# xiangli0608/Creating-2D-laser-slam-from-scratch

Measured on AMD Instinct MI355X. Metric: scan-matches/sec (1081-beam vs 2000x2000 grid), higher is better.
Workload: dtype u8

## Files before the change

### creating-2d-laser-slam-from-scratch_amd/api.py

```python
from __future__ import annotations

import ctypes as C
import os
import sys
import math
import weakref

import numpy as np

from . import build as _build

LSLAM_OK = 0
ERRORS = {
    -1: "LSLAM_ERR_INVALID_ARGUMENT",
    -2: "LSLAM_ERR_NO_DEVICE",
    -3: "LSLAM_ERR_INDEX_OUT_OF_RANGE",
    -4: "LSLAM_ERR_PROBABILITY_SEARCH",
    -5: "LSLAM_ERR_NO_BEST_POSE",
    -6: "LSLAM_ERR_HIP",
    -7: "LSLAM_ERR_SMEAR_DEVIATION",
    -8: "LSLAM_ERR_UNSUPPORTED",
}


# ... 218 lines not shown
    return LaserParams(laser.angle_min, laser.angle_max, laser.angle_increment, laser.range_min,
                       laser.range_max, range_threshold, *offset)


_LIB = None


def lib() -> C.CDLL:
    global _LIB
    if _LIB is not None:
        return _LIB
    path = os.environ.get("LSLAM_GPU_LIB") or _build.build_library()
    L = C.CDLL(str(path))
    vp, i32, dbl = C.c_void_p, C.c_int, C.c_double
    L.lslam_abi_version.restype = i32
    L.lslam_create.argtypes = [i32, C.POINTER(vp)]
    L.lslam_destroy.argtypes = [vp]
    L.lslam_last_error.restype = C.c_char_p
    L.lslam_last_error.argtypes = [vp]
    L.lslam_synchronize.argtypes = [vp]
    L.lslam_stream.restype = vp
    L.lslam_stream.argtypes = [vp]
    L.lslam_dev_alloc.argtypes = [vp, C.c_size_t, C.POINTER(vp)]
    L.lslam_dev_free.argtypes = [vp, vp]
    L.lslam_dev_upload.argtypes = [vp, vp, vp, C.c_size_t]
    L.lslam_dev_download.argtypes = [vp, vp, vp, C.c_size_t]
    L.lslam_profile_enable.argtypes = [vp, i32]
    L.lslam_profile_only.argtypes = [vp, C.c_char_p]
    L.lslam_profile_reset.argtypes = [vp]
    L.lslam_profile_read.argtypes = [vp, vp, i32]
    L.lslam_matcher_config_defaults.argtypes = [C.POINTER(MatcherConfig)]
    L.lslam_matcher_config_defaults.restype = None
    L.lslam_matcher_create.argtypes = [vp, C.POINTER(MatcherConfig), C.POINTER(LaserParams), C.POINTER(vp)]
    L.lslam_matcher_destroy.argtypes = [vp]
    L.lslam_matcher_destroy.restype = None
    L.lslam_matcher_num_beams.argtypes = [vp]
    L.lslam_matcher_grid_info.argtypes = [vp, vp, vp]
    L.lslam_matcher_get_grid_u8.argtypes = [vp, vp]
    L.lslam_matcher_get_kernel_u8.argtypes = [vp, vp]
    L.lslam_matcher_set_grid_u8.argtypes = [vp, vp, vp]
    L.lslam_matcher_set_grid_u8_dev.argtypes = [vp, vp, vp]
    L.lslam_matcher_grid_dev_ptr.restype = vp
    L.lslam_matcher_grid_dev_ptr.argtypes = [vp]
    L.lslam_sensor_pose_from_robot.argtypes = [C.POINTER(LaserParams), vp, vp]
    L.lslam_sensor_pose_from_robot.restype = None
    L.lslam_robot_pose_from_sensor.argtypes = [C.POINTER(LaserParams), vp, vp]
    L.lslam_robot_pose_from_sensor.restype = None
    L.lslam_matcher_set_base_scans.argtypes = [vp, i32, vp, i32, vp, vp]
    L.lslam_matcher_match_scan.argtypes = [vp, i32, vp, i32, vp, vp, vp, i32, i32, vp]
    L.lslam_matcher_match_batch.argtypes = [vp, i32, vp, i32, vp, i32, i32, vp]
    L.lslam_matcher_match_batch_dev_f32.argtypes = [vp, i32, vp, i32, vp, i32, i32, vp]
    L.lslam_matcher_match_batch_dev_f64.argtypes = [vp, i32, vp, i32, vp, i32, i32, vp]
    L.lslam_matcher_debug_lookup_table.argtypes = [vp, vp, vp, dbl, dbl, dbl, vp, C.POINTER(i32)]
    L.lslam_matcher_debug_coarse_sums.argtypes = [vp, vp, vp, vp, C.POINTER(i32), C.POINTER(i32),
                                                  C.POINTER(i32), i32]
    L.lslam_matcher_debug_coarse_sums_batch.argtypes = [vp, i32, vp, i32, vp, vp]
    L.lslam_matcher_debug_fine_sums_batch.argtypes = [vp, i32, vp, i32, vp, vp, vp, C.POINTER(i32), C.POINTER(i32), C.POINTER(i32)]
    L.lslam_matcher_debug_valid_mask.argtypes = [vp, vp, vp, vp, vp]
    L.lslam_frontend_create.argtypes = [vp, i32, dbl, dbl, dbl, C.POINTER(vp)]
    L.lslam_frontend_destroy.argtypes = [vp]
    L.lslam_frontend_destroy.restype = None
    L.lslam_frontend_reset.argtypes = [vp]
    L.lslam_frontend_process.argtypes = [vp, vp, i32, vp, C.POINTER(i32), vp, vp, C.POINTER(dbl)]
    L.lslam_frontend_running_scans.argtypes = [vp]
    L.lslam_frontend_config_defaults.argtypes = [C.POINTER(FrontEndConfig)]
    L.lslam_frontend_config_defaults.restype = None
# ... 1285 lines not shown
```

### creating-2d-laser-slam-from-scratch_amd/csrc/scan_matcher.hip

```cpp
#include <algorithm>
#include <atomic>
#include <chrono>
#include <cmath>
#include <cstdlib>
#include <cstring>
#include <type_traits>
#include <vector>

#include "common.hpp"
#include "karto_math.hpp"

using namespace lslam;

#if defined(LSLAM_EXP_SERIAL_PRIO)
#define LSLAM_SERIAL_BEGIN() __builtin_amdgcn_s_setprio(3)
#define LSLAM_SERIAL_END() __builtin_amdgcn_s_setprio(0)
#else
#define LSLAM_SERIAL_BEGIN()
#define LSLAM_SERIAL_END()
#endif

namespace {

LSLAM_STAMP_TABLE(g_sm_stamps)
// ... 965 lines not shown
  }
#pragma unroll
  for (int q = 0; q < kTile3Angles; q++) {
    uint32_t tot[9];
    tot[0] = wave_sum(e0[q] & 0xFFFFu), tot[1] = wave_sum(o01[q] & 0xFFFFu), tot[2] = wave_sum(e0[q] >> 16);
    tot[3] = wave_sum(e1[q] & 0xFFFFu), tot[4] = wave_sum(o01[q] >> 16), tot[5] = wave_sum(e1[q] >> 16);
    tot[6] = wave_sum(e2[q] & 0xFFFFu), tot[7] = wave_sum(o2[q]), tot[8] = wave_sum(e2[q] >> 16);
    uint32_t mine = 0;
#pragma unroll
    for (int c = 0; c < 9; c++)
      if (lane == c) mine = tot[c];
    if (lane < 9 && angle_on[q]) r_scan[(a0 + q) * 9 + lane] = (int32_t)mine;
  }
}

template <int kTile3Angles>
__global__ void __launch_bounds__(64)
k_resp_tile3(const uint4* __restrict__ tiles, int tile_cols, Geom g, PassCfg pc, const Lattice* __restrict__ lat,
             const double2* __restrict__ cossin, const double2* __restrict__ local, int32_t* __restrict__ resp, size_t resp_stride, int S) {
  const int w = blockIdx.x;
  const int xcd = w & 7, r = w >> 3;
  const int pairs = (pc.na + kTile3Angles - 1) / kTile3Angles;
  const int s = (r / pairs) * 8 + xcd;
  const int a0 = (r % pairs) * kTile3Angles;
  if (s >= S) return;
  resp_tile3_wave<kTile3Angles>(s, a0, (int)threadIdx.x, tiles, tile_cols, g, pc, lat, cossin, local, resp + (size_t)s * resp_stride);
}

constexpr int kPosChunk = 16;
#if !defined(LSLAM_TUNE_REDUCE_NARROW_MIN)
#define LSLAM_TUNE_REDUCE_NARROW_MIN 2048
#endif
constexpr int kReduceNarrowMinScans = LSLAM_TUNE_REDUCE_NARROW_MIN;
__device__ __forceinline__ void generic_item(const uint8_t* __restrict__ grid, const Geom& g, const PassCfg& pc,
                                             const Lattice& L, const double2* __restrict__ lp, int32_t* r, int a,
                                             int c, int lane) {
  const int np = pc.nx * pc.ny;
  const double angle = (L.center[2] - pc.ang_off) + (uint32_t)a * pc.ang_res;
  const double cosine = cos(angle), sine = sin(angle);
  int pos[kPosChunk];
#pragma unroll
  for (int q = 0; q < kPosChunk; q++) {
    int f = c * kPosChunk + q;
    pos[q] = f < np ? L.gx[f % pc.nx] + L.gy[f / pc.nx] * g.stride : -1;
  }
  int32_t acc[kPosChunk];
#pragma unroll
  for (int q = 0; q < kPosChunk; q++) acc[q] = 0;
  for (int b = lane; b < g.n_beams; b += 64) {
    double2 p = lp[b];
    if (isnan(p.x)) continue;
    int t = lookup_offset(p.x, p.y, cosine, sine, g.off_x, g.off_y, g.scale, g.stride);
#pragma unroll
    for (int q = 0; q < kPosChunk; q++) {
      long long idx = (long long)pos[q] + t;
      if (pos[q] >= 0 && idx >= 0 && idx < g.data_size) acc[q] += grid[idx];
    }
  }
#pragma unroll
  for (int q = 0; q < kPosChunk; q++) {
    int v = acc[q];
    for (int o = 32; o > 0; o >>= 1) v += __shfl_xor(v, o);
    int f = c * kPosChunk + q;
    if (lane == 0 && f < np) r[(size_t)a * np + f] = v;
  }
}

__global__ void __launch_bounds__(64)
k_resp_generic(const uint8_t* __restrict__ grid, Geom g, PassCfg pc, const Lattice* __restrict__ lat,
               const double2* __restrict__ local, int32_t* __restrict__ resp, size_t resp_stride, int S) {
  const int chunks = (pc.nx * pc.ny + kPosChunk - 1) / kPosChunk;
  const int per_scan = pc.na * chunks;
  const long long total = (long long)S * per_scan;
  for (long long w = blockIdx.x; w < total; w += gridDim.x) {
    const int s = (int)(w / per_scan), rem = (int)(w % per_scan);
    const Lattice& L = lat[s];
    if (!L.active || L.status != 0) continue;
    generic_item(grid, g, pc, L, local + (size_t)s * g.n_beams, resp + (size_t)s * resp_stride, rem / chunks,
                 rem % chunks, threadIdx.x);
  }
}

__device__ __forceinline__ void block_generic_fallback(const uint8_t* __restrict__ grid, const Geom& g,
                                                       const PassCfg& pc, const Lattice& L,
                                                       const double2* __restrict__ lp, int32_t* r, int fb_step,
                                                       int tid, int nthreads) {
  if (fb_step == 0 || (L.step_x == fb_step && L.step_y == fb_step)) return;
  const int chunks = (pc.nx * pc.ny + kPosChunk - 1) / kPosChunk;
  const int per_scan = pc.na * chunks;
  for (int w = tid >> 6; w < per_scan; w += nthreads >> 6) generic_item(grid, g, pc, L, lp, r, w / chunks, w % chunks, tid & 63);
  __syncthreads();
}

struct Cand {
  double x, y, angle;
};

__device__ __forceinline__ Cand cand_of(int k, const PassCfg& pc, const double* center) {
  int a = k % pc.na, c = k / pc.na;
  int xi = c % pc.nx, yi = c / pc.nx;
  Cand cd;
  cd.x = -pc.off_x + (uint32_t)xi * pc.res_x;
  cd.y = -pc.off_y + (uint32_t)yi * pc.res_y;
  cd.angle = (center[2] - pc.ang_off) + (uint32_t)a * pc.ang_res;
  return cd;
}

__device__ __forceinline__ double penalized(int32_t sum, const Cand& cd, const double* center, int n_beams,
                                            const SearchCfg& sc) {
  double r = response_of_sum(sum, n_beams, sc);
  if (sc.do_penalize && !double_equal(r, 0.0)) {
    double sd = ksq(cd.x) + ksq(cd.y);
    double dp = 1.0 - (kDistPenaltyGain * sd / sc.dvp);
    dp = dp > sc.min_dp ? dp : sc.min_dp;
    double sad = ksq(cd.angle - center[2]);
    double ap = 1.0 - (kAnglePenaltyGain * sad / sc.avp);
    ap = ap > sc.min_ap ? ap : sc.min_ap;
    r *= (dp * ap);
  }
  return r;
}

__device__ __forceinline__ double block_max(double v, double* sh, int tid, int nthreads) {
// ... 142 lines not shown
      cov[0] = kMaxVariance; cov[4] = kMaxVariance; cov[8] = 4 * ksq(pc.ang_res);
    } else {
      double axx = 0, axy = 0, ayy = 0, norm = 0;
      for (int c = 0; c < ncand; c++) {
        double rr = terms[4 * c];
        if (rr >= (best - 0.1)) {
          norm += rr;
          axx += terms[4 * c + 1];
          axy += terms[4 * c + 2];
          ayy += terms[4 * c + 3];
        }
      }
      if (norm > kTol) {
        double vxx = axx / norm, vxy = axy / norm, vyy = ayy / norm;
        double vthth = 4 * ksq(pc.ang_res);
        double min_xx = 0.1 * ksq(pc.res_x), min_yy = 0.1 * ksq(pc.res_y);
        vxx = vxx > min_xx ? vxx : min_xx;
        vyy = vyy > min_yy ? vyy : min_yy;
        double mult = 1.0 / best;
        cov[0] = vxx * mult; cov[1] = vxy * mult; cov[3] = vxy * mult; cov[4] = vyy * mult;
        cov[8] = vthth;
      }
      if (double_equal(cov[0], 0.0)) cov[0] = kMaxVariance;
      if (double_equal(cov[4], 0.0)) cov[4] = kMaxVariance;
    }
  }
  o.mean[0] = avg[0]; o.mean[1] = avg[1]; o.mean[2] = avg[2];
  for (int i = 0; i < 9; i++) o.cov[i] = cov[i];
  o.best = best > 1.0 ? 1.0 : best;
  o.expand = (use_expansion && o.status == 0 && pass_index < 3 && double_equal(o.best, 0.0)) ? 1 : 0;
  out[s] = o;
}

template <int NT>
__device__ __forceinline__ void reduce_coarse_lds_block(
    const int s, const int tid, const Geom& g, const PassCfg& pc, const SearchCfg& sc, Lattice* lat, int32_t* r,
    CoarseOut* __restrict__ out, int use_expansion, int pass_index, const uint8_t* __restrict__ grid,
    const double2* __restrict__ local, int fb_step, const PassCfg& fine_pc, double2* fine_cossin, int fine_step,
    int zero_fine_words, int parts, unsigned char* smem) {
  __shared__ double sh[NT];
  __shared__ double s_ap[kMaxAngles];
  __shared__ unsigned long long s_nz[4];
  __shared__ double s_avg[3];
  __shared__ int s_status, s_bad, s_ntie, s_wcnt[(NT + 63) / 64];
  const Lattice& L = lat[s];
  if (!L.active) return;
  if (L.status != 0) {
    if (tid == 0) { out[s].status = L.status; out[s].expand = 0; out[s].best = 0.0; }
    return;
  }
  LSLAM_PHASE_CLOCK(pck);
  block_generic_fallback(grid, g, pc, L, local + (size_t)s * g.n_beams, r, fb_step, tid, NT);
  const int ncand = pc.nx * pc.ny;
  const int total = ncand * pc.na;
  const int words = (total + 31) / 32;
  double* latmax = (double*)smem;
  double* probs = latmax + (size_t)parts * ncand;
  double* terms = probs + g.probs_side * g.probs_side;
  uint32_t* mask = (uint32_t*)(terms + 4 * ncand);
  int* cell = (int*)(mask + words);
  int* tie = cell + ncand;
  double* dpen = terms;
  const double center[3] = {L.center[0], L.center[1], L.center[2]};

  const double p_off_x = center[0] - pc.off_x, p_off_y = center[1] - pc.off_y;
  if (tid == 0) { s_bad = 0; s_ntie = 0; }
  for (int c = tid; c < ncand; c += NT) {
    const int xi = c % pc.nx, yi = c / pc.nx;
    const double x = -pc.off_x + (uint32_t)xi * pc.res_x;
    const double y = -pc.off_y + (uint32_t)yi * pc.res_y;
    const double sd = ksq(x) + ksq(y);
    double dp = 1.0 - (kDistPenaltyGain * sd / sc.dvp);
    dpen[c] = dp > sc.min_dp ? dp : sc.min_dp;
    const double wx = center[0] + x, wy = center[1] + y;
    const int gx = world_to_grid(wx, p_off_x, g.scale), gy = world_to_grid(wy, p_off_y, g.scale);
    cell[c] = (gx < 0 || gx >= g.probs_side || gy < 0 || gy >= g.probs_side) ? -1 : gy * g.probs_side + gx;
  }
  for (int a = tid; a < pc.na; a += NT) {
    const double angle = (center[2] - pc.ang_off) + (uint32_t)a * pc.ang_res;
    const double sad = ksq(angle - center[2]);
    double ap = 1.0 - (kAnglePenaltyGain * sad / sc.avp);
    s_ap[a] = ap > sc.min_ap ? ap : sc.min_ap;
  }
  for (int wd = tid; wd < words; wd += NT) mask[wd] = 0u;
  for (int c = tid; c < g.probs_side * g.probs_side; c += NT) probs[c] = 0.0;
  __syncthreads();
  LSLAM_PHASE_MARK(pck, 0);

  auto value_of = [&](int32_t sum, int c, int a) -> double {
    double v = response_of_sum(sum, g.n_beams, sc);
    if (sc.do_penalize && !double_equal(v, 0.0)) v *= (dpen[c] * s_ap[a]);
    return v;
  };
  double lm = -1.0;
  for (int idx = tid; idx < ncand * parts; idx += NT) {
    const int part = idx / ncand, c = idx - part * ncand;
    const int a_lo = part * pc.na / parts, a_hi = (part + 1) * pc.na / parts;
    double m = -1.0;
#if !defined(LSLAM_TUNE_REDUCE_BATCH)
#define LSLAM_TUNE_REDUCE_BATCH 11
#endif
    constexpr int kBatch = LSLAM_TUNE_REDUCE_BATCH;
    for (int a0 = a_lo; a0 < a_hi; a0 += kBatch) {
      int32_t rv[kBatch];
#pragma unroll
      for (int i = 0; i < kBatch; i++) rv[i] = a0 + i < a_hi ? r[(a0 + i) * ncand + c] : 0;
#pragma unroll
      for (int i = 0; i < kBatch; i++)
        if (a0 + i < a_hi) {
          const double v = value_of(rv[i], c, a0 + i);
          m = m > v ? m : v;
        }
    }
    latmax[(size_t)part * ncand + c] = m;
    lm = lm > m ? lm : m;
  }
  LSLAM_PHASE_MARK(pck, 1);
  const double best = block_max(lm, sh, tid, NT);
  LSLAM_PHASE_MARK(pck, 2);

  for (int c = tid; c < ncand; c += NT) {
    double m = latmax[c];
    for (int q = 1; q < parts; q++) m = m > latmax[(size_t)q * ncand + c] ? m : latmax[(size_t)q * ncand + c];
    latmax[c] = m;
    if (cell[c] < 0) s_bad = 1;
    else atomicMax((unsigned long long*)&probs[cell[c]], (unsigned long long)__double_as_longlong(m < 0.0 ? 0.0 : m));
    if (!(m + 2.0 * kTol < best)) tie[atomicAdd(&s_ntie, 1)] = c;
  }
  __syncthreads();
  for (int idx = tid, n = s_ntie * pc.na; idx < n; idx += NT) {
    const int c = tie[idx / pc.na], a = idx % pc.na;
    if (double_equal(value_of(r[a * ncand + c], c, a), best)) {
      const int k = c * pc.na + a;
      atomicOr(&mask[k >> 5], 1u << (k & 31));
    }
  }
  __syncthreads();
  for (int w0 = 0; w0 < 256; w0 += NT) {
    const int wd = w0 + tid;
    const unsigned long long nz = __ballot(wd < words && mask[wd] != 0u);
    if ((tid & 63) == 0 && wd < 256) s_nz[wd >> 6] = nz;
  }
  __syncthreads();
  LSLAM_PHASE_MARK(pck, 3);
  if (tid == 0) {
    LSLAM_SERIAL_BEGIN();
    int st = s_bad ? LSLAM_ERR_PROBABILITY_SEARCH : 0;
    double avg[3] = {0, 0, 0};
    if (st == 0) {
      double ax = 0, ay = 0, tx = 0, ty = 0;
      int cnt = 0;
      for (int wv = 0; wv < 4; wv++) {
        unsigned long long nzw = s_nz[wv];
        while (nzw) {
          const int wd = wv * 64 + (__ffsll((long long)nzw) - 1);
          nzw &= nzw - 1;
          uint32_t m = mask[wd];
          while (m) {
            const int bit = __ffs(m) - 1;
            m &= m - 1;
            const Cand cd = cand_of(wd * 32 + bit, pc, center);
            const double h = normalize_angle(cd.angle);
            ax += center[0] + cd.x;
            ay += center[1] + cd.y;
            double sn, cs;
            sincos(h, &sn, &cs);
            tx += cs;
            ty += sn;
            cnt++;
          }
        }
      }
      if (cnt == 0) {
        st = LSLAM_ERR_NO_BEST_POSE;
      } else {
        ax /= cnt; ay /= cnt; tx /= cnt; ty /= cnt;
        avg[0] = ax; avg[1] = ay; avg[2] = atan2(ty, tx);
      }
    }
    s_avg[0] = avg[0]; s_avg[1] = avg[1]; s_avg[2] = avg[2];
    s_status = st;
    LSLAM_SERIAL_END();
  }
  __syncthreads();
  LSLAM_PHASE_MARK(pck, 4);
  if (fine_cossin != nullptr && tid >= NT - 64) {
    const double center2[3] = {s_avg[0], s_avg[1], s_avg[2]};
    pass_setup_wave(s, tid - (NT - 64), g, fine_pc, center2, s_status == 0, lat, fine_cossin, fine_step);
  }
  const double dx = s_avg[0] - center[0], dy = s_avg[1] - center[1];
  const double thr = best - 0.1;
  int n_pass = 0;
  for (int c0 = 0; c0 < ncand; c0 += NT) {
    const int c = c0 + tid;
    double rr = 0.0, t1 = 0.0, t2 = 0.0, t3 = 0.0;
    bool pass = false;
    if (c < ncand) {
      const int xi = c % pc.nx, yi = c / pc.nx;
      const double x = -pc.off_x + (uint32_t)xi * pc.res_x;
      const double y = -pc.off_y + (uint32_t)yi * pc.res_y;
      rr = cell[c] >= 0 ? probs[cell[c]] : 0.0;
      t1 = (ksq(x - dx) * rr);
      t2 = ((x - dx) * (y - dy) * rr);
      t3 = (ksq(y - dy) * rr);
      pass = rr >= thr;
    }
    const unsigned long long bal = __ballot(pass);
    if ((tid & 63) == 0) s_wcnt[tid >> 6] = __popcll(bal);
    __syncthreads();
    int off = n_pass;
    for (int w = 0; w < (tid >> 6); w++) off += s_wcnt[w];
    for (int w = 0; w < (NT + 63) / 64; w++) n_pass += s_wcnt[w];
    if (pass) {
      const int k = off + __popcll(bal & ((1ull << (tid & 63)) - 1ull));
      terms[4 * k + 0] = rr; terms[4 * k + 1] = t1; terms[4 * k + 2] = t2; terms[4 * k + 3] = t3;
    }
    __syncthreads();
  }
  LSLAM_PHASE_MARK(pck, 5);
  if (tid == 0) {
    CoarseOut o;
    o.status = s_status;
    o.flags = pass_index > 0 ? 1 : 0;
    o.pad = 0;
    const double avg[3] = {s_avg[0], s_avg[1], s_avg[2]};
    double cov[9] = {1, 0, 0, 0, 1, 0, 0, 0, 1};
    if (o.status == 0) {
      if (best < kTol) {
        cov[0] = kMaxVariance; cov[4] = kMaxVariance; cov[8] = 4 * ksq(pc.ang_res);
      } else {
        double axx = 0, axy = 0, ayy = 0, norm = 0;
        int c = 0;
        for (; c + 4 <= n_pass; c += 4) {
          double q[16];
  #pragma unroll
          for (int i = 0; i < 16; i++) q[i] = terms[4 * c + i];
  #pragma unroll
          for (int i = 0; i < 4; i++) { norm += q[4 * i]; axx += q[4 * i + 1]; axy += q[4 * i + 2]; ayy += q[4 * i + 3]; }
        }
        for (; c < n_pass; c++) { norm += terms[4 * c]; axx += terms[4 * c + 1]; axy += terms[4 * c + 2]; ayy += terms[4 * c + 3]; }
        if (norm > kTol) {
          double vxx = axx / norm, vxy = axy / norm, vyy = ayy / norm;
          double vthth = 4 * ksq(pc.ang_res);
          double min_xx = 0.1 * ksq(pc.res_x), min_yy = 0.1 * ksq(pc.res_y);
          vxx = vxx > min_xx ? vxx : min_xx;
          vyy = vyy > min_yy ? vyy : min_yy;
          double mult = 1.0 / best;
          cov[0] = vxx * mult; cov[1] = vxy * mult; cov[3] = vxy * mult; cov[4] = vyy * mult;
          cov[8] = vthth;
        }
        if (double_equal(cov[0], 0.0)) cov[0] = kMaxVariance;
        if (double_equal(cov[4], 0.0)) cov[4] = kMaxVariance;
      }
    }
    o.mean[0] = avg[0]; o.mean[1] = avg[1]; o.mean[2] = avg[2];
    for (int i = 0; i < 9; i++) o.cov[i] = cov[i];
    o.best = best > 1.0 ? 1.0 : best;
    o.expand = (use_expansion && o.status == 0 && pass_index < 3 && double_equal(o.best, 0.0)) ? 1 : 0;
    out[s] = o;
  }
  for (int i = tid; i < zero_fine_words; i += NT) r[i] = 0;
  LSLAM_PHASE_MARK(pck, 6);
  LSLAM_PHASE_FLUSH(pck, g_sm_stamps, 3, (unsigned)(s * (NT >> 6) + (tid >> 6)), (tid & 63) == 0);
}

struct SpecArgs {
  const double* ranges;
  double pose[3];
  int* out;
  const double2* local;
};
__device__ __forceinline__ void anchor_spec_block(int n, const SpecArgs& sa, const Geom& g, unsigned char* smem);
template <int NT>
__global__ void __launch_bounds__(NT)
k_reduce_coarse_lds(Geom g, PassCfg pc, SearchCfg sc, Lattice* lat,
                    int32_t* resp, size_t resp_stride, CoarseOut* __restrict__ out,
                    int use_expansion, int pass_index, const uint8_t* __restrict__ grid,
                const double2* __restrict__ local, int fb_step, PassCfg fine_pc,
                    double2* fine_cossin, int fine_step, int zero_fine_words, int parts, SpecArgs spec) {
  extern __shared__ __align__(16) unsigned char smem[];
  if constexpr (NT == 1024) {
    if (spec.out && blockIdx.x + 1 == gridDim.x) {
      anchor_spec_block(g.n_beams, spec, g, smem);
      return;
    }
  }
  reduce_coarse_lds_block<NT>((int)blockIdx.x, (int)threadIdx.x, g, pc, sc, lat, resp + (size_t)blockIdx.x * resp_stride, out,
                              use_expansion, pass_index, grid, local, fb_step, fine_pc, fine_cossin, fine_step, zero_fine_words,
                              parts, smem);
}


__global__ void __launch_bounds__(256)
k_table_big(int S, Geom g, PassCfg pc, const Lattice* __restrict__ lat, const double2* __restrict__ local,
            int32_t* __restrict__ tbl, unsigned long long* __restrict__ best_bits) {
  const int b = blockIdx.x * blockDim.x + threadIdx.x;
  const int a = blockIdx.y, s = blockIdx.z;
  if (b == 0 && a == 0) best_bits[s] = 0ull;
  if (b >= g.n_beams) return;
  const Lattice& L = lat[s];
  int32_t v = kInvalidScan;
  if (L.active && L.status == 0) {
    const double angle = (L.center[2] - pc.ang_off) + (uint32_t)a * pc.ang_res;
    const double2 p = local[(size_t)s * g.n_beams + b];
    if (!isnan(p.x)) v = lookup_offset(p.x, p.y, cos(angle), sin(angle), g.off_x, g.off_y, g.scale, g.stride);
  }
  tbl[((size_t)s * pc.na + a) * g.n_beams + b] = v;
// ... 1566 lines not shown
  ~BusyGuard() {
    if (ok) m->busy.store(false);
  }
};
#define LSLAM_NOT_REENTRANT(m)                                                                                   \
  BusyGuard busy_guard(m);                                                                                       \
  if (!busy_guard.ok)                                                                                            \
    return (m)->ctx->fail(LSLAM_ERR_INVALID_ARGUMENT, "matcher used concurrently: a ScanMatcher instance is not " \
                                                      "re-entrant (one grid + one set of workspaces, Mapper.h:1273-1278)")

void arm_done_ticket(lslam_matcher* m) {
  if (!m->h_done) {
    if (hipHostMalloc((void**)&m->h_done, sizeof(int), hipHostMallocDefault) != hipSuccess) {
      (void)hipGetLastError();
      m->h_done = nullptr;
      return;
    }
    *m->h_done = 0;
  }
  m->arm_next = true;
}
int wait_record(lslam_matcher* m) {
  lslam_context* ctx = m->ctx;
  if (m->done_armed) {
    m->done_armed = false;
    if (spin_for_ticket(m->h_done, m->done_ticket)) return LSLAM_OK;
  }
  LSLAM_HIP(ctx, hipStreamSynchronize(ctx->stream));
  return LSLAM_OK;
}

int n_angles_of(double off, double res) { return lattice_count(off, res); }

PassCfg coarse_pass_cfg(const lslam_matcher* m, const Geom& g) {
  const double res = 1.0 / g.scale;
  PassCfg pc;
  pc.off_x = pc.off_y = 0.5 * ((double)g.probs_side - 1) * res;
  pc.res_x = pc.res_y = 2 * res;
  pc.ang_off = m->cfg.coarse_search_angle_offset;
  pc.ang_res = m->cfg.coarse_angle_resolution;
  pc.nx = lattice_count(pc.off_x, pc.res_x);
  pc.ny = lattice_count(pc.off_y, pc.res_y);
  pc.na = n_angles_of(pc.ang_off, pc.ang_res);
  pc.mode = 0;
  return pc;
}

template <typename RT>
int match_batch_impl(lslam_matcher* m, int S, const RT* d_ranges, int stride, const double* d_poses,
                     int do_penalize, int do_refine, lslam_match_result* d_out,
                     int32_t* dbg_coarse_sums , int force_generic) {
  lslam_context* ctx = m->ctx;
  if (!m->pipe_in_step) {
    int jrc = pipe_join(m);
    if (jrc) return jrc;
  }
  Geom g = m->g;
  const bool prep_was_done = m->prep_done;
  size_t prezeroed = m->resp_prezeroed;
  m->prep_done = false;
  m->resp_prezeroed = 0;
  int* done_flag = nullptr;
  int done_ticket = 0;
  m->done_armed = false;
  if (m->arm_next && S == 1 && S < kReduceNarrowMinScans && m->h_done) {
    done_flag = m->h_done;
    done_ticket = ++m->done_ticket;
    m->done_armed = true;
  }
  m->arm_next = false;
  const SpecArgs spec_req = m->spec_armed ? m->spec_req : SpecArgs{};
  m->spec_armed = false;
  m->spec_launched = false;
  if (S <= 0) return LSLAM_OK;
  LSLAM_HIP(ctx, hipSetDevice(ctx->device));
  if (g.n_beams == 0) {
    m->done_armed = false;
    launch(ctx, "result_no_readings", k_result_no_readings, dim3((S + 255) / 256), dim3(256), 0, S,
           d_poses, m->cfg.coarse_angle_resolution, d_out);
// ... 82 lines not shown
      m->ptile_dirty = false;
    }
    return true;
  };
  auto tiles4_possible = [&]() -> bool {
    return g.n_beams <= 16384 && !m->tile_failed &&
           (unsigned long long)g.data_size * 4ull + (1ull << 24) < (1ull << 32);
  };
  auto ensure_tiles4 = [&]() -> bool {
    if (!tiles4_possible()) return false;
    if (!m->d_tiles) {
      m->tile_cols = g.stride / 2;
      m->tile_rows = (g.height + 1) / 2 + kTileYPad / 2 + 1;
      m->tile_rows += m->tile_rows & 1;
      if (hipMalloc((void**)&m->d_tiles, (size_t)((m->tile_cols + 3) / 4) * 4 * m->tile_rows * sizeof(uint4)) != hipSuccess) {
        (void)hipGetLastError();
        m->d_tiles = nullptr;
        m->tile_failed = true;
        return false;
      }
    }
    if (m->tile_dirty) {
      launch(ctx, "tile4", k_tile4, dim3((m->tile_cols + 255) / 256, m->tile_rows), dim3(256), 0,
             (const uint8_t*)m->d_grid, g.stride, g.data_size, m->d_tiles, m->tile_cols, m->tile_rows);
      m->tile_dirty = false;
    }
    return true;
  };
  auto reduce_lds = [&](const PassCfg& p, bool cache) -> size_t {
    size_t total = (size_t)p.nx * p.ny * p.na;
    return (cache ? total * 8 : 0) + (size_t)p.nx * p.ny * (8 + 32 + 4) + (size_t)g.probs_side * g.probs_side * 8 +
           ((total + 31) / 32) * 4 + 16;
  };
  auto reduce_parts = [&](const PassCfg& p, int nt) -> int { return std::max(1, std::min(8, nt / (p.nx * p.ny))); };
  auto reduce_lds_nocache = [&](const PassCfg& p, int parts) -> size_t {
    size_t total = (size_t)p.nx * p.ny * p.na;
    return (size_t)p.nx * p.ny * (8 * parts + 32 + 4 + 4) + (size_t)g.probs_side * g.probs_side * 8 + ((total + 31) / 32) * 4 + 16;
  };
  int fb_step = 0;
  bool fine_prezeroed = false;
  auto run_responses = [&](const PassCfg& p, int step, const char* name) -> int {
    const int variant = force_generic ? 0 : (p.nx <= 4 && p.ny <= 4) ? 1 : (p.nx <= 12) ? 2 : (p.nx <= 16) ? 3 : 0;
    fb_step = variant ? step : 0;
    if (!setup_done)
      launch(ctx, "pass_setup", k_pass_setup, dim3(S), dim3(64), 0, S, g, p, d_poses,
             (const CoarseOut*)m->d_coarse.p, m->d_lat.p, m->d_cossin.p, step);
    setup_done = false;
    const long long waves = (long long)((S + 7) / 8) * 8 * p.na;
    bool tiled = variant == 1 && step == 1 && p.nx == 3 && p.ny == 3 && waves >= kTileMinWaves && tiles4_possible();
    if (tiled) tiled = ensure_tiles4();
    if (tiled) {
      m->form_launches[LSLAM_FORM_FINE_TILE3]++;
#define LSLAM_TILE3_ARGS                                                                                                \
  (const uint4*)m->d_tiles, m->tile_cols, g, p, (const Lattice*)m->d_lat.p, (const double2*)m->d_cossin.p,              \
      (const double2*)m->d_local.p, m->d_resp.p, resp_stride, S
      if (S >= kTile3ManyMinScans)
        launch(ctx, "resp_tile_fine", k_resp_tile3<kTile3ManyAngles>,
               dim3((unsigned)((long long)((S + 7) / 8) * 8 * ((p.na + kTile3ManyAngles - 1) / kTile3ManyAngles))), dim3(64), 0,
               LSLAM_TILE3_ARGS);
      else
        launch(ctx, "resp_tile_fine", k_resp_tile3<1>, dim3((unsigned)waves), dim3(64), 0, LSLAM_TILE3_ARGS);
#undef LSLAM_TILE3_ARGS
    } else if (variant) {
      int slices = 1;
      while (slices < 8 && waves * slices < 2048) slices *= 2;
      while ((g.n_beams + 64 * slices - 1) / (64 * slices) > kMaxBeamsPerLane) slices *= 2;
      if (slices > 1) {
        if (step == 1 && fine_prezeroed) fine_prezeroed = false;
        else if (prezeroed >= (size_t)S * resp_stride) prezeroed = 0;
        else LSLAM_HIP(ctx, hipMemsetAsync(m->d_resp.p, 0, (size_t)S * resp_stride * sizeof(int32_t), ctx->stream));
// ... 518 lines not shown
  c->smear_deviation = 0.03;
  c->range_threshold = 12.0;
  c->coarse_search_angle_offset = 20.0 * kPi180;
  c->coarse_angle_resolution = 2.0 * kPi180;
  c->fine_search_angle_offset = 0.2 * kPi180;
  c->distance_variance_penalty = 0.3 * 0.3;
  c->angle_variance_penalty = (20.0 * kPi180) * (20.0 * kPi180);
  c->minimum_distance_penalty = 0.5;
  c->minimum_angle_penalty = 0.9;
  c->use_response_expansion = 0;
  c->reserved = 0;
}

void lslam_sensor_pose_from_robot(const lslam_laser* l, const double robot[3], double sensor[3]) {
  SensorXform t = sensor_xform(robot[0], robot[1], robot[2]);
  double rx, ry;
  rot_apply(t.rot, l->offset_x, l->offset_y, l->offset_heading, rx, ry);
  sensor[0] = t.tx + rx;
  sensor[1] = t.ty + ry;
  sensor[2] = normalize_angle(l->offset_heading + t.th);
}

void lslam_robot_pose_from_sensor(const lslam_laser* l, const double sensor[3], double robot[3]) {
  double len = sqrt(ksq(l->offset_x) + ksq(l->offset_y));
  double angleoffset = atan2(l->offset_y, l->offset_x);
  double ch = normalize_angle(sensor[2]);
  double wx = len * cos(ch + angleoffset - l->offset_heading);
  double wy = len * sin(ch + angleoffset - l->offset_heading);
  robot[0] = sensor[0] - wx;
  robot[1] = sensor[1] - wy;
  robot[2] = normalize_angle(sensor[2] - l->offset_heading);
}

int lslam_matcher_create(lslam_context* ctx, const lslam_matcher_config* cfg, const lslam_laser* laser,
                         lslam_matcher** out) {
  if (!ctx || !cfg || !laser || !out) return LSLAM_ERR_INVALID_ARGUMENT;
  *out = nullptr;
  if (!(cfg->resolution > 0) || !(cfg->search_size > 0) || cfg->smear_deviation < 0 || !(cfg->range_threshold > 0))
    return ctx->fail(LSLAM_ERR_INVALID_ARGUMENT, "invalid matcher parameters (ScanMatcher::Create -> NULL)");
  if (!(cfg->smear_deviation >= 0.5 * cfg->resolution && cfg->smear_deviation <= 10 * cfg->resolution))
    return ctx->fail(LSLAM_ERR_SMEAR_DEVIATION, "smear deviation must be within [%g, %g]", 0.5 * cfg->resolution,
                     10 * cfg->resolution);
  if (!(laser->angular_resolution != 0.0))
    return ctx->fail(LSLAM_ERR_INVALID_ARGUMENT, "laser angular_resolution must be non-zero");
  lslam_matcher* m = new lslam_matcher();
  m->ctx = ctx;
  m->cfg = *cfg;
  m->laser = *laser;
  Geom& g = m->g;
  g.n_beams = (int)(uint32_t)kround((laser->maximum_angle - laser->minimum_angle) / laser->angular_resolution);
  uint32_t side = (uint32_t)(kround(cfg->search_size / cfg->resolution) + 1);
  uint32_t margin = (uint32_t)ceil(cfg->range_threshold / cfg->resolution);
  int grid_size = (int)(side + 2 * margin);
  int half = (int)kround(2.0 * cfg->smear_deviation / cfg->resolution);
  g.border = half + 1;
  g.roi_w = g.roi_h = grid_size;
  g.width = g.height = grid_size + 2 * g.border;
  g.stride = (g.width + 7) & ~7;
  if (g.stride > kMaxGridSide || g.height > kMaxGridSide) {
    delete m;
    return ctx->fail(LSLAM_ERR_UNSUPPORTED, "correlation grid of %dx%d cells exceeds the built limit %d per side",
                     g.width, g.height, kMaxGridSide);
  }
  g.data_size = g.stride * g.height;
  g.scale = 1.0 / cfg->resolution;
  g.off_x = g.off_y = 0.0;
// ... 649 lines not shown
```

### include/lslam_gpu.h

```cpp
#ifndef LSLAM_GPU_H
#define LSLAM_GPU_H

#include <stddef.h>
#include <stdint.h>

#ifdef __cplusplus
extern "C" {
#endif

#define LSLAM_ABI_VERSION 5

typedef enum lslam_status {
  LSLAM_OK = 0,
  LSLAM_ERR_INVALID_ARGUMENT = -1,
  LSLAM_ERR_NO_DEVICE = -2,
  LSLAM_ERR_INDEX_OUT_OF_RANGE = -3,
  LSLAM_ERR_PROBABILITY_SEARCH = -4,
  LSLAM_ERR_NO_BEST_POSE = -5,
  LSLAM_ERR_HIP = -6,
  LSLAM_ERR_SMEAR_DEVIATION = -7,
  LSLAM_ERR_UNSUPPORTED = -8,
  LSLAM_ERR_NO_DATA = -9
} lslam_status;

// ... 49 lines not shown
  double response;
  double covariance[9];
  int32_t status;
  int32_t flags;
} lslam_match_result;

void lslam_matcher_config_defaults(lslam_matcher_config* cfg);

int lslam_matcher_create(lslam_context* ctx, const lslam_matcher_config* cfg,
                         const lslam_laser* laser, lslam_matcher** out);
void lslam_matcher_destroy(lslam_matcher* m);

int lslam_matcher_num_beams(const lslam_matcher* m);
int lslam_matcher_grid_info(const lslam_matcher* m, int32_t out[8], double offset_xy[2]);
int lslam_matcher_get_grid_u8(lslam_matcher* m, uint8_t* out_host);
int lslam_matcher_get_kernel_u8(lslam_matcher* m, uint8_t* out_host);
int lslam_matcher_set_grid_u8(lslam_matcher* m, const uint8_t* grid_host, const double offset_xy[2]);
int lslam_matcher_set_grid_u8_dev(lslam_matcher* m, const uint8_t* grid_dev, const double offset_xy[2]);
void* lslam_matcher_grid_dev_ptr(lslam_matcher* m);

enum { LSLAM_OPT_ROW_OCCUPANCY = 1, LSLAM_OPT_COLLECT_STATS = 2, LSLAM_OPT_LDS_STAGED = 3, LSLAM_OPT_PIPELINE_DEPTH = 4,
       LSLAM_OPT_STEP_KERNEL = 5, LSLAM_OPT_STEP_MIN_SCANS = 6, LSLAM_OPT_ROWS_WAVES = 7, LSLAM_OPT_CHECK_OUTPUT_REUSE = 8, LSLAM_OPT_LONE_KERNEL = 9 };
int lslam_matcher_get_option(const lslam_matcher* m, int option);
int lslam_matcher_flush(lslam_matcher* m);
int64_t lslam_matcher_pipelined_steps(const lslam_matcher* m);
int64_t lslam_matcher_step_kernel_launches(const lslam_matcher* m);
int64_t lslam_matcher_lone_kernel_launches(const lslam_matcher* m);
enum { LSLAM_FORM_GENERIC = 0, LSLAM_FORM_ROWS_LINEAR = 1, LSLAM_FORM_ROWS_TILED = 2, LSLAM_FORM_ROWS_MULTIWAVE = 3,
       LSLAM_FORM_ROWS_LDS_STAGED = 4, LSLAM_FORM_ROWS_STATS_LINEAR = 5, LSLAM_FORM_ROWS_STATS_TILED = 6,
       LSLAM_FORM_ROWS_STATS_LDS_STAGED = 7, LSLAM_FORM_BIG = 8, LSLAM_FORM_FINE_ROWS = 9, LSLAM_FORM_FINE_TILE3 = 10,
       LSLAM_FORM_COUNT = 11 };
int lslam_matcher_coarse_form_launches(const lslam_matcher* m, int64_t out[LSLAM_FORM_COUNT]);
int lslam_debug_lone_sync(lslam_matcher* m, unsigned* out128);
int lslam_matcher_set_option(lslam_matcher* m, int option, int value);
int lslam_matcher_read_stats(lslam_matcher* m, uint64_t out[4]);
int lslam_matcher_read_beam_stats(lslam_matcher* m, uint64_t out[4]);

void lslam_sensor_pose_from_robot(const lslam_laser* laser, const double robot[3], double sensor[3]);
void lslam_robot_pose_from_sensor(const lslam_laser* laser, const double sensor[3], double robot[3]);

int lslam_matcher_set_base_scans(lslam_matcher* m, int n_scans, const double* ranges,
                                 int ranges_stride, const double* sensor_poses,
                                 const double center_pose[3]);

int lslam_matcher_match_scan(lslam_matcher* m, int n_base, const double* base_ranges,
                             int ranges_stride, const double* base_sensor_poses,
                             const double* query_ranges, const double query_sensor_pose[3],
                             int do_penalize, int do_refine, lslam_match_result* out);

int lslam_matcher_match_batch(lslam_matcher* m, int n_scans, const double* ranges,
                              int ranges_stride, const double* sensor_poses, int do_penalize,
                              int do_refine, lslam_match_result* out);
int lslam_matcher_match_batch_dev_f32(lslam_matcher* m, int n_scans, const float* ranges_dev,
                                      int ranges_stride, const double* sensor_poses_dev,
                                      int do_penalize, int do_refine,
                                      lslam_match_result* out_dev);
int lslam_matcher_match_batch_dev_f64(lslam_matcher* m, int n_scans, const double* ranges_dev,
                                      int ranges_stride, const double* sensor_poses_dev,
                                      int do_penalize, int do_refine,
                                      lslam_match_result* out_dev);

typedef struct lslam_scan_cache lslam_scan_cache;
int lslam_scan_cache_create(lslam_context* ctx, const lslam_laser* laser, lslam_scan_cache** out);
void lslam_scan_cache_destroy(lslam_scan_cache* cache);
int lslam_scan_cache_put(lslam_scan_cache* cache, int64_t scan_id, const double* ranges);
int lslam_scan_cache_contains(const lslam_scan_cache* cache, int64_t scan_id);
// ... 261 lines not shown
```

Before: 7.262 million.

## Shrink coarse-reduce LDS footprint and tune narrow-block occupancy

Overlays the dpen/latmax/terms regions of the coarse reduce kernel's shared memory and computes the layout through a shared ReduceLds struct, so the dynamic LDS size drops. It also shrinks the static block-max scratch to one slot per wave, and stores best in shared memory to free registers. For 128-thread blocks it uses a smaller fallback chunk and a smaller batch and sets a waves-per-EU hint, all to raise occupancy. The overlapping buffers add aliasing risk if their lifetimes overlap, and a debug entry point is added to report the LDS size.

New measurement: 7.482 million (median of 6 runs). +3.0%, better.

```diff
diff --git a/creating-2d-laser-slam-from-scratch_amd/api.py b/creating-2d-laser-slam-from-scratch_amd/api.py
--- a/creating-2d-laser-slam-from-scratch_amd/api.py
+++ b/creating-2d-laser-slam-from-scratch_amd/api.py
@@ -274,6 +274,8 @@
     L.lslam_matcher_config_defaults.argtypes = [C.POINTER(MatcherConfig)]
     L.lslam_matcher_config_defaults.restype = None
     L.lslam_matcher_create.argtypes = [vp, C.POINTER(MatcherConfig), C.POINTER(LaserParams), C.POINTER(vp)]
+    L.lslam_debug_reduce_lds_bytes.argtypes = [C.POINTER(MatcherConfig), i32, C.POINTER(i32 * 3)]
+    L.lslam_debug_reduce_lds_bytes.restype = i32
     L.lslam_matcher_destroy.argtypes = [vp]
     L.lslam_matcher_destroy.restype = None
     L.lslam_matcher_num_beams.argtypes = [vp]
diff --git a/creating-2d-laser-slam-from-scratch_amd/csrc/scan_matcher.hip b/creating-2d-laser-slam-from-scratch_amd/csrc/scan_matcher.hip
--- a/creating-2d-laser-slam-from-scratch_amd/csrc/scan_matcher.hip
+++ b/creating-2d-laser-slam-from-scratch_amd/csrc/scan_matcher.hip
@@ -1021,36 +1021,37 @@
 #define LSLAM_TUNE_REDUCE_NARROW_MIN 2048
 #endif
 constexpr int kReduceNarrowMinScans = LSLAM_TUNE_REDUCE_NARROW_MIN;
+template <int CH = kPosChunk>
 __device__ __forceinline__ void generic_item(const uint8_t* __restrict__ grid, const Geom& g, const PassCfg& pc,
                                              const Lattice& L, const double2* __restrict__ lp, int32_t* r, int a,
                                              int c, int lane) {
   const int np = pc.nx * pc.ny;
   const double angle = (L.center[2] - pc.ang_off) + (uint32_t)a * pc.ang_res;
   const double cosine = cos(angle), sine = sin(angle);
-  int pos[kPosChunk];
-#pragma unroll
-  for (int q = 0; q < kPosChunk; q++) {
-    int f = c * kPosChunk + q;
+  int pos[CH];
+#pragma unroll
+  for (int q = 0; q < CH; q++) {
+    int f = c * CH + q;
     pos[q] = f < np ? L.gx[f % pc.nx] + L.gy[f / pc.nx] * g.stride : -1;
   }
-  int32_t acc[kPosChunk];
-#pragma unroll
-  for (int q = 0; q < kPosChunk; q++) acc[q] = 0;
+  int32_t acc[CH];
+#pragma unroll
+  for (int q = 0; q < CH; q++) acc[q] = 0;
   for (int b = lane; b < g.n_beams; b += 64) {
     double2 p = lp[b];
     if (isnan(p.x)) continue;
     int t = lookup_offset(p.x, p.y, cosine, sine, g.off_x, g.off_y, g.scale, g.stride);
 #pragma unroll
-    for (int q = 0; q < kPosChunk; q++) {
+    for (int q = 0; q < CH; q++) {
       long long idx = (long long)pos[q] + t;
       if (pos[q] >= 0 && idx >= 0 && idx < g.data_size) acc[q] += grid[idx];
     }
   }
 #pragma unroll
-  for (int q = 0; q < kPosChunk; q++) {
+  for (int q = 0; q < CH; q++) {
     int v = acc[q];
     for (int o = 32; o > 0; o >>= 1) v += __shfl_xor(v, o);
-    int f = c * kPosChunk + q;
+    int f = c * CH + q;
     if (lane == 0 && f < np) r[(size_t)a * np + f] = v;
   }
 }
@@ -1070,14 +1071,15 @@
   }
 }
 
+template <int CH = kPosChunk>
 __device__ __forceinline__ void block_generic_fallback(const uint8_t* __restrict__ grid, const Geom& g,
                                                        const PassCfg& pc, const Lattice& L,
                                                        const double2* __restrict__ lp, int32_t* r, int fb_step,
                                                        int tid, int nthreads) {
   if (fb_step == 0 || (L.step_x == fb_step && L.step_y == fb_step)) return;
-  const int chunks = (pc.nx * pc.ny + kPosChunk - 1) / kPosChunk;
+  const int chunks = (pc.nx * pc.ny + CH - 1) / CH;
   const int per_scan = pc.na * chunks;
-  for (int w = tid >> 6; w < per_scan; w += nthreads >> 6) generic_item(grid, g, pc, L, lp, r, w / chunks, w % chunks, tid & 63);
+  for (int w = tid >> 6; w < per_scan; w += nthreads >> 6) generic_item<CH>(grid, g, pc, L, lp, r, w / chunks, w % chunks, tid & 63);
   __syncthreads();
 }
 
@@ -1286,16 +1288,28 @@
   out[s] = o;
 }
 
+struct ReduceLds {
+  int probs, mask, cell, tie, bytes;
+  __host__ __device__ ReduceLds(int ncand, int na, int probs_side, int parts) {
+    const int words = (ncand * na + 31) / 32;
+    probs = (1 + parts > 4 ? 1 + parts : 4) * ncand * 8;
+    mask = probs + probs_side * probs_side * 8;
+    cell = mask + words * 4;
+    tie = cell + ncand * 4;
+    bytes = tie + ncand * 4 + 16;
+  }
+};
+constexpr int kReduceNarrowChunk = 4;
 template <int NT>
 __device__ __forceinline__ void reduce_coarse_lds_block(
     const int s, const int tid, const Geom& g, const PassCfg& pc, const SearchCfg& sc, Lattice* lat, int32_t* r,
     CoarseOut* __restrict__ out, int use_expansion, int pass_index, const uint8_t* __restrict__ grid,
     const double2* __restrict__ local, int fb_step, const PassCfg& fine_pc, double2* fine_cossin, int fine_step,
     int zero_fine_words, int parts, unsigned char* smem) {
-  __shared__ double sh[NT];
+  __shared__ double sh[NT / 64];
   __shared__ double s_ap[kMaxAngles];
   __shared__ unsigned long long s_nz[4];
-  __shared__ double s_avg[3];
+  __shared__ double s_avg[3], s_best;
   __shared__ int s_status, s_bad, s_ntie, s_wcnt[(NT + 63) / 64];
   const Lattice& L = lat[s];
   if (!L.active) return;
@@ -1304,17 +1318,19 @@
     return;
   }
   LSLAM_PHASE_CLOCK(pck);
-  block_generic_fallback(grid, g, pc, L, local + (size_t)s * g.n_beams, r, fb_step, tid, NT);
+  block_generic_fallback<NT == 128 ? kReduceNarrowChunk : kPosChunk>(grid, g, pc, L, local + (size_t)s * g.n_beams, r, fb_step,
+                                                                     tid, NT);
   const int ncand = pc.nx * pc.ny;
   const int total = ncand * pc.na;
   const int words = (total + 31) / 32;
-  double* latmax = (double*)smem;
-  double* probs = latmax + (size_t)parts * ncand;
-  double* terms = probs + g.probs_side * g.probs_side;
-  uint32_t* mask = (uint32_t*)(terms + 4 * ncand);
-  int* cell = (int*)(mask + words);
-  int* tie = cell + ncand;
-  double* dpen = terms;
+  const ReduceLds lds(ncand, pc.na, g.probs_side, parts);
+  double* dpen = (double*)smem;
+  double* latmax = dpen + ncand;
+  double* terms = (double*)smem;
+  double* probs = (double*)(smem + lds.probs);
+  uint32_t* mask = (uint32_t*)(smem + lds.mask);
+  int* cell = (int*)(smem + lds.cell);
+  int* tie = (int*)(smem + lds.tie);
   const double center[3] = {L.center[0], L.center[1], L.center[2]};
 
   const double p_off_x = center[0] - pc.off_x, p_off_y = center[1] - pc.off_y;
@@ -1354,7 +1370,10 @@
 #if !defined(LSLAM_TUNE_REDUCE_BATCH)
 #define LSLAM_TUNE_REDUCE_BATCH 11
 #endif
-    constexpr int kBatch = LSLAM_TUNE_REDUCE_BATCH;
+#if !defined(LSLAM_TUNE_REDUCE_BATCH_NARROW)
+#define LSLAM_TUNE_REDUCE_BATCH_NARROW 7
+#endif
+    constexpr int kBatch = NT == 128 ? LSLAM_TUNE_REDUCE_BATCH_NARROW : LSLAM_TUNE_REDUCE_BATCH;
     for (int a0 = a_lo; a0 < a_hi; a0 += kBatch) {
       int32_t rv[kBatch];
 #pragma unroll
@@ -1370,7 +1389,7 @@
     lm = lm > m ? lm : m;
   }
   LSLAM_PHASE_MARK(pck, 1);
-  const double best = block_max(lm, sh, tid, NT);
+  const double best0 = block_max(lm, sh, tid, NT);
   LSLAM_PHASE_MARK(pck, 2);
 
   for (int c = tid; c < ncand; c += NT) {
@@ -1379,12 +1398,12 @@
     latmax[c] = m;
     if (cell[c] < 0) s_bad = 1;
     else atomicMax((unsigned long long*)&probs[cell[c]], (unsigned long long)__double_as_longlong(m < 0.0 ? 0.0 : m));
-    if (!(m + 2.0 * kTol < best)) tie[atomicAdd(&s_ntie, 1)] = c;
+    if (!(m + 2.0 * kTol < best0)) tie[atomicAdd(&s_ntie, 1)] = c;
   }
   __syncthreads();
   for (int idx = tid, n = s_ntie * pc.na; idx < n; idx += NT) {
     const int c = tie[idx / pc.na], a = idx % pc.na;
-    if (double_equal(value_of(r[a * ncand + c], c, a), best)) {
+    if (double_equal(value_of(r[a * ncand + c], c, a), best0)) {
       const int k = c * pc.na + a;
       atomicOr(&mask[k >> 5], 1u << (k & 31));
     }
@@ -1399,6 +1418,7 @@
   LSLAM_PHASE_MARK(pck, 3);
   if (tid == 0) {
     LSLAM_SERIAL_BEGIN();
+    s_best = best0;
     int st = s_bad ? LSLAM_ERR_PROBABILITY_SEARCH : 0;
     double avg[3] = {0, 0, 0};
     if (st == 0) {
@@ -1443,7 +1463,7 @@
     pass_setup_wave(s, tid - (NT - 64), g, fine_pc, center2, s_status == 0, lat, fine_cossin, fine_step);
   }
   const double dx = s_avg[0] - center[0], dy = s_avg[1] - center[1];
-  const double thr = best - 0.1;
+  const double thr = s_best - 0.1;
   int n_pass = 0;
   for (int c0 = 0; c0 < ncand; c0 += NT) {
     const int c = c0 + tid;
@@ -1474,6 +1494,7 @@
   LSLAM_PHASE_MARK(pck, 5);
   if (tid == 0) {
     CoarseOut o;
+    const double best = s_best;
     o.status = s_status;
     o.flags = pass_index > 0 ? 1 : 0;
     o.pad = 0;
@@ -1526,7 +1547,7 @@
 };
 __device__ __forceinline__ void anchor_spec_block(int n, const SpecArgs& sa, const Geom& g, unsigned char* smem);
 template <int NT>
-__global__ void __launch_bounds__(NT)
+__global__ void __launch_bounds__(NT) __attribute__((amdgpu_waves_per_eu(NT == 128 ? 8 : NT / 256 > 0 ? NT / 256 : 1, 8)))
 k_reduce_coarse_lds(Geom g, PassCfg pc, SearchCfg sc, Lattice* lat,
                     int32_t* resp, size_t resp_stride, CoarseOut* __restrict__ out,
                     int use_expansion, int pass_index, const uint8_t* __restrict__ grid,
@@ -3159,19 +3180,21 @@
 
 int n_angles_of(double off, double res) { return lattice_count(off, res); }
 
-PassCfg coarse_pass_cfg(const lslam_matcher* m, const Geom& g) {
+PassCfg coarse_pass_cfg(const lslam_matcher_config& cfg, const Geom& g) {
   const double res = 1.0 / g.scale;
   PassCfg pc;
   pc.off_x = pc.off_y = 0.5 * ((double)g.probs_side - 1) * res;
   pc.res_x = pc.res_y = 2 * res;
-  pc.ang_off = m->cfg.coarse_search_angle_offset;
-  pc.ang_res = m->cfg.coarse_angle_resolution;
+  pc.ang_off = cfg.coarse_search_angle_offset;
+  pc.ang_res = cfg.coarse_angle_resolution;
   pc.nx = lattice_count(pc.off_x, pc.res_x);
   pc.ny = lattice_count(pc.off_y, pc.res_y);
   pc.na = n_angles_of(pc.ang_off, pc.ang_res);
   pc.mode = 0;
   return pc;
 }
+PassCfg coarse_pass_cfg(const lslam_matcher* m, const Geom& g) { return coarse_pass_cfg(m->cfg, g); }
+int reduce_parts_of(int ncand, int nt) { return std::max(1, std::min(8, nt / ncand)); }
 
 template <typename RT>
 int match_batch_impl(lslam_matcher* m, int S, const RT* d_ranges, int stride, const double* d_poses,
@@ -3320,10 +3343,9 @@
     return (cache ? total * 8 : 0) + (size_t)p.nx * p.ny * (8 + 32 + 4) + (size_t)g.probs_side * g.probs_side * 8 +
            ((total + 31) / 32) * 4 + 16;
   };
-  auto reduce_parts = [&](const PassCfg& p, int nt) -> int { return std::max(1, std::min(8, nt / (p.nx * p.ny))); };
+  auto reduce_parts = [&](const PassCfg& p, int nt) -> int { return reduce_parts_of(p.nx * p.ny, nt); };
   auto reduce_lds_nocache = [&](const PassCfg& p, int parts) -> size_t {
-    size_t total = (size_t)p.nx * p.ny * p.na;
-    return (size_t)p.nx * p.ny * (8 * parts + 32 + 4 + 4) + (size_t)g.probs_side * g.probs_side * 8 + ((total + 31) / 32) * 4 + 16;
+    return (size_t)ReduceLds(p.nx * p.ny, p.na, g.probs_side, parts).bytes;
   };
   int fb_step = 0;
   bool fine_prezeroed = false;
@@ -3908,6 +3930,16 @@
   robot[2] = normalize_angle(sensor[2] - l->offset_heading);
 }
 
+int lslam_debug_reduce_lds_bytes(const lslam_matcher_config* cfg, int threads, int dims[3]) {
+  if (!cfg || !(cfg->resolution > 0.0) || (threads != 128 && threads != 256 && threads != 1024)) return -1;
+  Geom g{};
+  g.scale = 1.0 / cfg->resolution;
+  g.probs_side = (int)(uint32_t)(kround(cfg->search_size / cfg->resolution) + 1);
+  const PassCfg pc = coarse_pass_cfg(*cfg, g);
+  if (dims) { dims[0] = pc.nx; dims[1] = pc.ny; dims[2] = pc.na; }
+  return ReduceLds(pc.nx * pc.ny, pc.na, g.probs_side, reduce_parts_of(pc.nx * pc.ny, threads)).bytes;
+}
+
 int lslam_matcher_create(lslam_context* ctx, const lslam_matcher_config* cfg, const lslam_laser* laser,
                          lslam_matcher** out) {
   if (!ctx || !cfg || !laser || !out) return LSLAM_ERR_INVALID_ARGUMENT;
diff --git a/include/lslam_gpu.h b/include/lslam_gpu.h
--- a/include/lslam_gpu.h
+++ b/include/lslam_gpu.h
@@ -105,6 +105,7 @@
        LSLAM_FORM_COUNT = 11 };
 int lslam_matcher_coarse_form_launches(const lslam_matcher* m, int64_t out[LSLAM_FORM_COUNT]);
 int lslam_debug_lone_sync(lslam_matcher* m, unsigned* out128);
+int lslam_debug_reduce_lds_bytes(const lslam_matcher_config* cfg, int threads, int dims[3]);
 int lslam_matcher_set_option(lslam_matcher* m, int option, int value);
 int lslam_matcher_read_stats(lslam_matcher* m, uint64_t out[4]);
 int lslam_matcher_read_beam_stats(lslam_matcher* m, uint64_t out[4]);
```
